# anibali/dsnt-pose2d

Measured on AMD Instinct MI355X. Metric: images/sec (train step, 256x256, 16 joints), higher is better.
Workload: dtype f32; 1 GPU; hg2 + DSNT + JS reg, 256x256 -> 64x64x16, batch 32 per GPU, RMSprop lr 2.5e-4, train step fwd+loss+bwd+optim; global_batch=32, parallelism=dp1, launches_fwd=212

## Files before the change

### dsnt-pose2d_amd/csrc/fwd1.h

```cpp
#pragma once
#include "conv_split.h"

struct Fwd1Plan {
    int ok;
    int cfg;
    int chunks;
    int nstages;
    int spw;
    int nwg;
    int lds;
};
Fwd1Plan dsnt_fwd1_plan(const dsnt_conv_geom* g, bool share);
```

### dsnt-pose2d_amd/csrc/fwd1.hip

```cpp
#include "fwd1.h"
#include <stdlib.h>

typedef unsigned f1_u32x4 __attribute__((ext_vector_type(4)));
typedef float f32x4 __attribute__((ext_vector_type(4)));

struct Fwd1P {
    const float* x; const float* in_scale; const float* in_shift; int in_relu;
    const unsigned short* wq; long wq_stride;
    const float* a_bound; const float* w_bound;
    const float* bias; const float* res; float* y; float* stats;
    OutBoundsP ob;
    int M, Cout, nstages, spw;
};

template <int KK, int CW, int NWV, bool PRO, bool RES>
__global__ __launch_bounds__(64 * NWV, 2) void fwd1_kernel(Fwd1P p) {
    constexpr int CC = 16 * CW * NWV;
    constexpr int NTHR = 64 * NWV;
    constexpr int KS = KK / 32;
    constexpr int PITCH = KK * 2 + 32;
    constexpr int PL = 32 * PITCH;
    constexpr int IMG = 2 * PL;
    constexpr int WLO = CC * PITCH;
    constexpr int K4 = KK / 4;
    constexpr int U = 32 * K4 / NTHR;
    constexpr int RSTEP = NTHR / K4;
    static_assert(U >= 1 && U * NTHR == 32 * K4, "staging units per thread");
    const unsigned OOB = 0xF0000000u;
    extern __shared__ __attribute__((aligned(16))) unsigned char f1_smem[];
    unsigned char* img = f1_smem;
    unsigned char* wlo = f1_smem + 2 * IMG;
// ... 94 lines not shown
        const int c = col0 + c0 + 16 * cw + lc;
        cb[cw] = p.bias ? p.bias[c] : 0.f;
        asc[cw] = p.ob.amax_bn ? p.ob.amax_scale[c] : 0.f;
        ash[cw] = p.ob.amax_bn ? p.ob.amax_shift[c] : 0.f;
    }
    const float am2lo = p.ob.amax_relu ? 0.f : -__builtin_inff();
    __syncthreads();
    transform(0);
    issue(s0 + 1);
    __syncthreads();

    float s1a[CW], s2a[CW];
#pragma unroll
    for (int cw = 0; cw < CW; ++cw) { s1a[cw] = 0.f; s2a[cw] = 0.f; }
    float am = 0.f, am2 = 0.f;
    const unsigned a_lane = (unsigned)(lc * PITCH + 16 * lg);
    const unsigned w_lane = (unsigned)(2 * IMG + (c0 + lc) * PITCH + 16 * lg);

    auto stage = [&](const int s) {
        const int buf = (s - s0) & 1;
        transform(buf ^ 1);
        issue(s + 2);
        __builtin_amdgcn_sched_barrier(0);
        const unsigned ib = (unsigned)(buf * IMG);
#pragma unroll
        for (int rt = 0; rt < 2; ++rt) {
            f32x4 acc[CW];
#pragma unroll
            for (int cw = 0; cw < CW; ++cw) acc[cw] = (f32x4){0.f, 0.f, 0.f, 0.f};
#pragma unroll
            for (int ks = 0; ks < KS; ++ks) {
                const unsigned ao = ib + (unsigned)(rt * 16 * PITCH + 64 * ks) + a_lane;
                const f16x8 d1 = *reinterpret_cast<const f16x8*>(f1_smem + ao);
                const f16x8 d2 = *reinterpret_cast<const f16x8*>(f1_smem + ao + PL);
#pragma unroll
                for (int cw = 0; cw < CW; ++cw) {
                    const f16x8 b2 = *reinterpret_cast<const f16x8*>(f1_smem + w_lane + cw * 16 * PITCH + 64 * ks);
                    acc[cw] = __builtin_amdgcn_mfma_f32_16x16x32_f16(d2, whi[ks][cw], acc[cw], 0, 0, 0);
                    acc[cw] = __builtin_amdgcn_mfma_f32_16x16x32_f16(d1, b2, acc[cw], 0, 0, 0);
                    acc[cw] = __builtin_amdgcn_mfma_f32_16x16x32_f16(d1, whi[ks][cw], acc[cw], 0, 0, 0);
                }
            }
            const unsigned obase = (unsigned)(s * 32 + 16 * rt) * (unsigned)ld * 4u + ylane;
#pragma unroll
            for (int cw = 0; cw < CW; ++cw) {
#pragma unroll
                for (int r = 0; r < 4; ++r) {
                    float v = acc[cw][r] * osc + cb[cw];
                    if (RES) v += rv[rt][cw][r];
                    __builtin_amdgcn_raw_buffer_store_b32(__float_as_uint(v), yr, obase + (unsigned)(cw * 64), (unsigned)(r * ld * 4), 0);
                    am = fmaxf(am, fabsf(v));
                    am2 = fmaxf(am2, fabsf(fmaxf(fmaf(v, asc[cw], ash[cw]), am2lo)));
                    s1a[cw] += v;
                    s2a[cw] = fmaf(v, v, s2a[cw]);
                }
            }
            issue_r(rt, s + 1);
        }
        __syncthreads();
    };
    stage(s0);
    for (int s = s0 + 1; s < s1; ++s) stage(s);

    if (p.stats) {
#pragma unroll
        for (int cw = 0; cw < CW; ++cw) {
            float a = s1a[cw], b = s2a[cw];
            a += __shfl_xor(a, 16, 64); b += __shfl_xor(b, 16, 64);
            a += __shfl_xor(a, 32, 64); b += __shfl_xor(b, 32, 64);
            if (lg == 0) {
                p.stats[((size_t)wg * 2 + 0) * ld + col0 + c0 + 16 * cw + lc] = a;
                p.stats[((size_t)wg * 2 + 1) * ld + col0 + c0 + 16 * cw + lc] = b;
            }
        }
    }
    if (p.ob.amax) amax_commit(am, p.ob.amax);
    if (p.ob.amax_bn) amax_commit(am2, p.ob.amax_bn, 1);
}

static int f1_enabled = -1;
struct F1Cfg { int cin, cout, cw, nwv, chunks; };
static const F1Cfg f1_cfgs[] = {
    {256, 128, 1, 8, 1},
    {128, 256, 2, 8, 1},
    {128, 128, 1, 8, 1},
    {64, 64, 1, 4, 1},
    {64, 128, 1, 8, 1},
    {256, 256, 1, 8, 2},
};

Fwd1Plan dsnt_fwd1_plan(const dsnt_conv_geom* g, bool share) {
    Fwd1Plan pl;
// ... 13 lines not shown
    const F1Cfg& c = f1_cfgs[cfg];
    const int cus = dsnt_device_cus();
    const int nstages = (int)(M / 32);
    int nwg = cus * (c.nwv == 4 ? 2 : 1) / c.chunks;
    if (share) nwg = nwg / 2 > 0 ? nwg / 2 : 1;
    if (c.chunks > 1) nwg = nwg / 8 * 8 > 0 ? nwg / 8 * 8 : nwg;
    if (nwg > nstages) nwg = nstages;
    const int spw = (nstages + nwg - 1) / nwg;
    nwg = (nstages + spw - 1) / spw;
    const int pitch = c.cin * 2 + 32;
    pl.ok = 1; pl.cfg = cfg; pl.nstages = nstages; pl.spw = spw; pl.nwg = nwg; pl.chunks = c.chunks;
    pl.lds = 2 * 2 * 32 * pitch + 16 * c.cw * c.nwv * pitch + 2 * c.cin * 4;
    return pl;
}

template <int KK, int CW, int NWV, bool PRO, bool RES>
static void f1_launch_k(const Fwd1Plan& pl, const Fwd1P& p, hipStream_t st) {
    DSNT_SET_MAX_LDS((fwd1_kernel<KK, CW, NWV, PRO, RES>), pl.lds);
    DSNT_LAUNCH((fwd1_kernel<KK, CW, NWV, PRO, RES>), dim3(pl.nwg, pl.chunks), dim3(64 * NWV), pl.lds, st, p);
}
template <int KK, int CW, int NWV>
static void f1_launch_cfg(const Fwd1Plan& pl, const Fwd1P& p, hipStream_t st) {
    const bool pro = p.in_scale != nullptr, res = p.res != nullptr;
    if (pro) { if (res) f1_launch_k<KK, CW, NWV, true, true>(pl, p, st); else f1_launch_k<KK, CW, NWV, true, false>(pl, p, st); }
    else { if (res) f1_launch_k<KK, CW, NWV, false, true>(pl, p, st); else f1_launch_k<KK, CW, NWV, false, false>(pl, p, st); }
}

extern "C" int dsnt_conv1x1_fwd_ok(const dsnt_conv_geom* g) { return dsnt_fwd1_plan(g, false).ok; }
extern "C" int dsnt_conv1x1_fwd_stats_rows(const dsnt_conv_geom* g, int in_relu_flags) {
    return dsnt_fwd1_plan(g, (in_relu_flags & DSNT_CONV_SHARE_CHIP) != 0).nwg;
// ... 16 lines not shown
    if (int e = out_bounds_fill(p.ob, tail, "dsnt_conv1x1_fwd_f16x3")) return e;
    p.x = x; p.in_scale = in_scale; p.in_shift = in_shift; p.in_relu = in_relu & 1;
    p.wq = (const unsigned short*)w_planes; p.wq_stride = plane_stride; p.a_bound = a_bound; p.w_bound = w_bound;
    p.bias = bias; p.res = res1; p.y = y; p.stats = stats_partial;
    p.M = g->N * g->H * g->W; p.Cout = g->Cout; p.nstages = pl.nstages; p.spw = pl.spw;
    hipStream_t st = (hipStream_t)stream;
    switch (pl.cfg) {
    case 0: case 5: f1_launch_cfg<256, 1, 8>(pl, p, st); break;
    case 1: f1_launch_cfg<128, 2, 8>(pl, p, st); break;
    case 2: f1_launch_cfg<128, 1, 8>(pl, p, st); break;
    case 3: f1_launch_cfg<64, 1, 4>(pl, p, st); break;
    default: f1_launch_cfg<64, 1, 8>(pl, p, st); break;
    }
    DSNT_CHECK_LAUNCH("dsnt_conv1x1_fwd_f16x3");
}
```

### dsnt-pose2d_amd/dsnt/_lib.py

```python
import ctypes as C
import os

import torch

_HERE = os.path.dirname(os.path.abspath(__file__))
LIB_PATH = os.environ.get('DSNT_HIP_LIB') or os.path.join(os.path.dirname(_HERE), 'csrc', 'libdsnt_hip.so')

P = C.c_void_p
I = C.c_int
L = C.c_int64
F = C.c_float
D = C.c_double


class ConvGeom(C.Structure):
    _fields_ = [(n, C.c_int) for n in
                ('N', 'H', 'W', 'Cin', 'Ho', 'Wo', 'Cout', 'R', 'S', 'stride', 'pad', 'dil')]


GP = C.POINTER(ConvGeom)


class BnBwdEpilogue(C.Structure):
    _fields_ = [('x', C.c_void_p), ('scale', C.c_void_p), ('shift', C.c_void_p), ('mean', C.c_void_p),
# ... 61 lines not shown
    'dsnt_conv_fwd_bf16x6_ex': [P, P, L, P, P, P, P, I, P, P, P, GP, BP, TP, P],
    'dsnt_conv_pack_dgrad': [P, P, I, I, I, I, P],
    'dsnt_conv_pack_dgrad_all': [P, I, P, P, P, L, P],
    'dsnt_conv_fwd_bf16x6': [P, P, L, P, P, P, P, I, P, P, P, GP, P],
    'dsnt_split_bf16x3': [P, P, L, P],
    'dsnt_conv_fwd_f16x3_ex': [P, P, L, P, P, P, P, P, P, I, P, P, P, GP, BP, TP, P],
    'dsnt_conv_fwd_f16x3_stream': [P, P, L, P, P, P, P, P, P, I, P, P, P, GP, BP, TP, P],
    'dsnt_amax': [P, L, P, P],
    'dsnt_split_f16x2': [P, P, L, L, P, P],
    'dsnt_f16_prep_weights': [P, I, I, P],
    'dsnt_f16_prep_bn_bounds': [P, I, P],
    'dsnt_conv_wgrad': [P, P, P, I, P, P, P, P, I, GP, P],
    'dsnt_conv_wgrad_bf16x6': [P, P, P, I, P, P, P, P, I, GP, P],
    'dsnt_conv_wgrad_f16x3': [P, P, P, I, P, P, P, P, I, P, P, GP, P],
    'dsnt_conv1x1_fwd_f16x3': [P, P, L, P, P, P, P, P, P, I, P, P, GP, TP, P],
    'dsnt_conv1x1_bwd_f16x3': [BP, P, AP, P, L, P, P, P, P, P, P, P, I, GP, P],
    'dsnt_conv_dgrad_f16x3_stream_apply': [P, AP, P, P, L, P, P, P, P, I, GP, BP, TP, P],
    'dsnt_wgrad_reduce_all': [P, I, I, P],
    'dsnt_conv_wgrad_group': [P, I, I, P],
    'dsnt_bn_stats': [P, P, L, I, P],
    'dsnt_bn_finalize': [P, I, L, I, P, P, P, P, F, F, I, P, P, P, P, P],
    'dsnt_bn_act_fwd': [P, P, P, I, P, L, I, P],
    'dsnt_bn_act_bwd_reduce': [P, P, P, P, P, P, I, P, L, I, P],
    'dsnt_bn_bwd_finalize': [P, I, L, I, P, P, I, P, P],
    'dsnt_bn_bwd_finalize_bound': [P, I, L, I, P, P, I, P, P, P, P, P],
    'dsnt_bn_eval_prep': [P, I, P],
    'dsnt_bn_act_bwd_apply': [P, P, P, P, P, P, P, I, P, I, L, I, P],
    'dsnt_bn_act_bwd_apply_amax': [P, P, P, P, P, P, P, I, P, I, L, I, P, P],
    'dsnt_bn_act_bwd_apply_pro': [P, P, P, P, P, P, P, I, P, P, I, P, I, P, I, L, I, P, P],
    'dsnt_stem4_fwd_f16x3': [P, P, L, P, P, P, P, P, GP, TP, P],
# ... 70 lines not shown
    'dsnt_conv_bf16x6_ok': (I, [GP]),
    'dsnt_conv_wgrad_bf16x6_ok': (I, [GP]),
    'dsnt_conv_wgrad_splits': (I, [GP]),
    'dsnt_conv_wgrad_halo_ok': (I, [GP]),
    'dsnt_conv_f16x3_route': (I, [GP, I]),
    'dsnt_conv_fwd_stream_ok': (I, [GP]),
    'dsnt_conv_fwd_stream_form': (I, [GP, I]),
    'dsnt_conv_dgrad_strided_ok': (I, [GP]),
    'dsnt_conv_dgrad_strided_tiles': (I, [GP]),
    'dsnt_conv_fwd_pro_ok': (I, [GP, I, I]),
    'dsnt_conv_wgrad_f16x3_splits': (I, [GP, I]),
    'dsnt_conv_wgrad_f16x3_ws_floats': (L, [GP, I]),
    'dsnt_conv_wgrad_ws_floats': (L, [GP]),
    'dsnt_conv1x1_fwd_ok': (I, [GP]),
    'dsnt_conv1x1_fwd_stats_rows': (I, [GP, I]),
    'dsnt_stem4_fwd_ok': (I, [GP]),
    'dsnt_stem4_fwd_stats_rows': (I, [GP]),
    'dsnt_conv1x1_bwd_ok': (I, [GP]),
    'dsnt_conv1x1_bwd_splits': (I, [GP, I]),
    'dsnt_conv1x1_bwd_ws_floats': (L, [GP, I]),
    'dsnt_conv_wgrad_desc_bytes': (I, []),
    'dsnt_conv_wgrad_desc': (I, [P, P, P, I, P, P, GP, P]),
    'dsnt_conv_wgrad_desc_f16x3': (I, [P, P, P, I, P, P, P, P, GP, P]),
    'dsnt_debug_set_timeline': (I, [P, I]),
}

_lib = None


def load():
# ... 50 lines not shown
```

### dsnt-pose2d_amd/dsnt/engine.py

```python
import ctypes as C
import os

import torch

from . import _lib
from ._lib import ConvGeom, BnBwdEpilogue, BnTail, BnPrologue, BnBwdApply

BN_EPS = 1e-5
BN_MOMENTUM = 0.1


class Act:
    __slots__ = ('buf', 'N', 'H', 'W', 'C', '_grad', 'stats', 'name', 'grad_amax', 'amax_tail', 'fold_ok',
                 'pending_apply', 'uses', 'gives_away', 'is_branch', 'grad_shared', 'pending_add', 'base', 'base_amax')

    def __init__(self, buf, name=''):
        self.buf = buf
        self.N, self.H, self.W, self.C = buf.shape
        self._grad = None
        self.base, self.base_amax = None, None
        self.stats = None
        self.amax_tail = None
        self.grad_amax = None
        self.fold_ok = False
        self.pending_apply = None
        self.uses = 0
        self.gives_away = False
        self.is_branch = False
        self.grad_shared = False
        self.pending_add = None
        self.name = name

    @property
    def M(self):
        return self.N * self.H * self.W

# ... 57 lines not shown
        self.side_stream = None
        self.wgrad_stream = None
        self.side_lanes = (1, 3)
        self.n_lanes = 3 + len(self.side_lanes) - 1
        self.chain_lanes = (0,) + self.side_lanes
        self.more_streams = ()
        self.wgrad_lane = 2 if (self.use_lanes and os.environ.get('DSNT_WGRAD_LANE', '1') != '0') else None
        self.wgrad_lane_rows = int(os.environ.get('DSNT_X_WGRAD_LANE_ROWS', '16000'))
        self.wgrad_lane_res = False
        self.wgrad_lane_from = self.chain_lanes
        self.conv3s = 'conv3s' not in os.environ.get('DSNT_OFF', '').replace('+', ',').split(',')
        self.bwd1 = 'bwd1' not in os.environ.get('DSNT_OFF', '').replace('+', ',').split(',')
        self.fwd1 = 'fwd1' not in os.environ.get('DSNT_OFF', '').replace('+', ',').split(',')
        self.fold3 = 'fold3' not in os.environ.get('DSNT_OFF', '').replace('+', ',').split(',')
        self.fold3_rows = int(os.environ.get('DSNT_X_FOLD3_ROWS', '16384'))
        self.stem4 = 'stem4' not in os.environ.get('DSNT_OFF', '').replace('+', ',').split(',')
        self.stage = os.environ.get('DSNT_STAGE', '0') == '1'
        self.stage_min_run = int(os.environ.get('DSNT_X_STAGE_MIN_RUN', '3'))
        self.stage_max_vgrid = int(os.environ.get('DSNT_X_STAGE_MAX_VGRID', '512'))
        self.stage_grid = int(os.environ.get('DSNT_X_STAGE_GRID', '64'))
        self.stage_census = []
        self._f16_w_stream = {}
        self.conv_share = True
        self.wgrad_share = True
        self._x = dict(kv.split('=') for kv in os.environ.get('DSNT_X', '').split(',') if '=' in kv)
        self.wgrad_narrow = self._x.get('wgrad_narrow', '1')
        self.share_grads = self._x.get('share_grads', '1') != '0'
        self.defer_res = self._x.get('defer_res', '1') != '0'
        self.flush_points = self._x.get('flush_points', '1') != '0'
        self.prep_split = self._x.get('prep_split', '1') != '0'
# ... 126 lines not shown
            return None
        got = self._famax_bn_of.get(id(t))
        if got is not None:
            return got[1] if got[0] is n else None
        slot = self._famax_slot()
        t.amax_bn, t.amax_scale, t.amax_shift = slot.data_ptr(), n.scale.data_ptr(), n.shift.data_ptr()
        t.amax_relu = 1 if n.relu else 0
        self._famax_bn_of[id(t)] = (n, slot)
        self._keep.append(t)
        return slot

    def f16_bn_bound_bwd(self, n):
        assert n.abound is not None, 'fp16x3 backward needs the BN bound its forward conv registered'
        return n.abound

    _PREP_CONSUMERS = ('dsnt_conv_fwd_f16x3_ex', 'dsnt_conv_fwd_f16x3_stream', 'dsnt_conv1x1_fwd_f16x3', 'dsnt_stem4_fwd_f16x3',
                       'dsnt_conv_fwd_bf16x6_ex', 'dsnt_conv_fwd_bf16x6')

    def emit_f16_prep(self, pos, head=()):
        side = 1 if (self.use_lanes and self.prep_on_side_lane and self.training) else 0
        saved, self.fwd = self.fwd, []
        saved_lane, self.lane = self.lane, side
        for fn, args, name, _ in head:
            self.fwd.append((fn, args, name, side))
        if self._f16_w_rows:
            t = torch.tensor(self._f16_w_rows, dtype=torch.int64).to(self.device)
            self._keep.append(t)
            self.f('dsnt_f16_prep_weights', t, len(self._f16_w_rows), 7)
        if self._f16_bn_rows:
            t = torch.tensor(self._f16_bn_rows, dtype=torch.int64).to(self.device)
            self._keep.append(t)
# ... 485 lines not shown
                self.b('dsnt_bn_act_bwd_apply_pro_base', da, x.buf, n.scale, n.shift, n.mean, n.invstd, part, tiles,
                       bn.ggamma, bn.gbeta, acc_p, coef, relu, base, buf, x.M, bn.C, x.grad_amax)
            else:
                self.b('dsnt_bn_act_bwd_apply_pro', da, x.buf, n.scale, n.shift, n.mean, n.invstd, part, tiles,
                       bn.ggamma, bn.gbeta, acc_p, coef, relu, buf, acc, x.M, bn.C, x.grad_amax)
        elif base is not None:
            self.b('dsnt_bn_act_bwd_apply_base', da, x.buf, n.scale, n.shift, n.mean, n.invstd, coef, relu,
                   base, buf, x.M, bn.C, x.grad_amax)
        elif x.grad_amax is not None:
            self.b('dsnt_bn_act_bwd_apply_amax', da, x.buf, n.scale, n.shift, n.mean, n.invstd, coef, relu,
                   buf, acc, x.M, bn.C, x.grad_amax)
        else:
            self.b('dsnt_bn_act_bwd_apply', da, x.buf, n.scale, n.shift, n.mean, n.invstd, coef, relu,
                   buf, acc, x.M, bn.C)

    def conv(self, src, p, res1=None, res2=None, want_stats=False, need_input_grad=True, name=''):
        normed = isinstance(src, Normed)
        x = src.x if normed else src
        g = self.geom(x, p)
        y = self.act(x.N, g.Ho, g.Wo, p.Cout, name)
        x.uses += 1
        for r in (res1, res2):
            if r is not None:
                r.uses += 1
                y.gives_away = True
        sc = src.scale if normed else None
        sh = src.shift if normed else None
        relu = 1 if (normed and src.relu) else 0
        if normed:
            self.check_lane(src)
        part, tail = None, None
        use6 = self._use6(g) and p.wq is not None
        x_amax_pre = None
        if use6 and p.wq16 is not None and p.R == 1 and res2 is None and self.fwd1:
            x_amax_pre = self.operand_amax_bn(src) if normed else self.operand_amax(x)
        f1 = bool(use6 and self.use_f16x3 and p.wq16 is not None and p.R == 1 and res2 is None and self.fwd1 and
                  ((self.training and normed) or x_amax_pre is not None) and self.lib.dsnt_conv1x1_fwd_ok(C.byref(g)))
        f1_shr = 2 if (f1 and self.lane != 0 and self.conv_share) else 0
        s4 = bool(use6 and self.use_f16x3 and self.stem4 and p.wq16 is not None and not normed and res1 is None and res2 is None and
                  self.lib.dsnt_stem4_fwd_ok(C.byref(g)))
        if want_stats and self.training:
            bm = 128 if use6 else self.lib.dsnt_conv_fwd_bm(C.byref(g))
            tiles = (self.lib.dsnt_conv1x1_fwd_stats_rows(C.byref(g), f1_shr) if f1 else
                     self.lib.dsnt_stem4_fwd_stats_rows(C.byref(g)) if s4 else (y.M + bm - 1) // bm)
            part = self.empty(tiles, 2, p.Cout)
            y.stats = (part, tiles)
        if use6 and self.use_f16x3:
            y.amax_tail = tail = BnTail()
        r1 = res1.buf if res1 is not None else None
        r2 = res2.buf if res2 is not None else None
        if self.use_f16x3 and self.training and normed:
            self.f16_bn_bound(src)
        x_amax = x_amax_pre
        if x_amax is None and use6 and p.wq16 is not None:
            x_amax = self.operand_amax_bn(src) if normed else self.operand_amax(x)
        use16 = use6 and self.use_f16x3 and p.wq16 is not None and ((self.training and normed) or x_amax is not None)
        if normed and (use16 or use6):
            self.materialize(src)
        if use16:
            st = self.stream_ok(p, g, y.M, res2)
            self.f16_weights(p, stream=st)
            ab = self.f16_bn_bound(src) if (normed and self.training) else x_amax
            shr = 2 if ((st or p.R == 1) and self.lane != 0 and self.conv_share) else 0
            if f1:
                e = self.f('dsnt_conv1x1_fwd_f16x3', x.buf, p.wq16, p.wq_stride, p.wb, ab, p.b, y.buf, sc, sh, relu | f1_shr, r1,
                           part, g, tail)
            elif s4:
                e = self.f('dsnt_stem4_fwd_f16x3', x.buf, p.wq16, p.wq_stride, p.wb, ab, p.b, y.buf, part, g, tail)
            else:
                e = self.f('dsnt_conv_fwd_f16x3_stream' if st else 'dsnt_conv_fwd_f16x3_ex', x.buf, p.wq16, p.wq_stride, p.wb, ab,
                           p.b, y.buf, sc, sh, relu | shr, r1, r2, part, g, None, tail)
            self.f16_uses.append((e, dict(kind='fwd', name=name, x=x.buf, sc=sc, sh=sh, relu=relu, a_bound=ab,
                                          w=p.w, w_bound=p.wb)))
        elif use6:
            self.f('dsnt_conv_fwd_bf16x6_ex', x.buf, p.wq, p.wq_stride, p.b, y.buf, sc, sh, relu, r1, r2, part, g,
                   None, tail)
        elif normed and src.pending is not None and self.lib.dsnt_conv_fwd_pro_ok(C.byref(g), src.pending[1], src.bn.C):
            spart, stiles = src.pending
            src.pending = None
# ... 300 lines not shown
            y.amax_tail = BnTail() if big else None
            self.f('dsnt_bn_act_fwd_stats', x.buf, n.scale, n.shift, 1 if n.relu else 0, y.buf, part, x.M, x.C, y.amax_tail)
            y.stats = (part, tiles)
        elif not self.training and big:
            y.amax_tail = BnTail()
            self.f('dsnt_bn_act_fwd_stats', x.buf, n.scale, n.shift, 1 if n.relu else 0, y.buf, None, x.M, x.C, y.amax_tail)
        else:
            self.f('dsnt_bn_act_fwd', x.buf, n.scale, n.shift, 1 if n.relu else 0, y.buf, x.M, x.C)
        if self.record:
            def backward():
                self._norm_backward(n, y.grad)
            self.on_backward(backward)
        return y

    def maxpool2(self, x, name=''):
        y = self.act(x.N, x.H // 2, x.W // 2, x.C, name)
        x.uses += 1
        idx = self.empty(x.N, x.H // 2, x.W // 2, x.C, dtype=torch.uint8)
        if self.training and self.fuse_op_stats:
            tiles = (y.M + 127) // 128
            part = self.empty(tiles, 2, x.C)
            y.amax_tail = BnTail() if (self.use_f16x3 and y.M >= self.bf16x6_min_rows) else None
            self.f('dsnt_maxpool2_fwd_stats', x.buf, y.buf, idx, part, x.N, x.H, x.W, x.C, y.amax_tail)
            y.stats = (part, tiles)
        elif not self.training and self.use_f16x3 and y.M >= self.bf16x6_min_rows:
            y.amax_tail = BnTail()
            self.f('dsnt_maxpool2_fwd_stats', x.buf, y.buf, idx, None, x.N, x.H, x.W, x.C, y.amax_tail)
        else:
            self.f('dsnt_maxpool2_fwd', x.buf, y.buf, idx, x.N, x.H, x.W, x.C)
        if self.record:
            def backward():
                add, x.pending_add = x.pending_add, None
                buf, acc = self.grad_target(x, amax=True, take_add=True)
                if add is not None:
# ... 128 lines not shown
```

### dsnt-pose2d_amd/dsnt/hourglass.py

```python
import os

import torch
import torch.nn as nn
from torch.autograd import Function

from . import _lib
from .engine import Tape, ConvParams, BnParams

EXPANSION = 2


def _ceil4(n):
    return (n + 3) // 4 * 4


class Arena:

    def __init__(self, module, device):
        self.device = device
        self.publish_scale = 1.0
        slots, off = [], 0
        skip = tuple(getattr(module, 'tape_exclude', ()))
        named = [(n, p) for n, p in module.named_parameters() if not (skip and n.startswith(skip))]
        bucket_of = getattr(module, 'param_bucket', lambda name: 0)
# ... 336 lines not shown
    expansion = EXPANSION

    def __init__(self, inplanes, planes, stride=1, downsample=None):
        super().__init__()
        self.bn1 = nn.BatchNorm2d(inplanes)
        self.conv1 = nn.Conv2d(inplanes, planes, kernel_size=1, bias=True)
        self.bn2 = nn.BatchNorm2d(planes)
        self.conv2 = nn.Conv2d(planes, planes, kernel_size=3, stride=stride, padding=1, bias=True)
        self.bn3 = nn.BatchNorm2d(planes)
        self.conv3 = nn.Conv2d(planes, planes * 2, kernel_size=1, bias=True)
        self.relu = nn.ReLU(inplace=True)
        self.downsample = downsample
        self.stride = stride
        self.out_channels = planes * 2

    def trace(self, t, x, P):
        skip = x
        if self.downsample is not None:
            skip = t.conv(x, P.conv(self.downsample[0]), name='ds')
        y = t.conv(t.norm(x, P.bn(self.bn1)), P.conv(self.conv1), want_stats=True, name='c1')
        y = t.conv(t.norm(y, P.bn(self.bn2)), P.conv(self.conv2), want_stats=True, name='c2')
        return t.conv(t.norm(y, P.bn(self.bn3)), P.conv(self.conv3), res1=skip, want_stats=True,
                      name='c3')


def _trace_seq(seq, t, x, P):
    for m in seq:
        x = m.trace(t, x, P)
    return x


class Hourglass(TapeModule):

    def __init__(self, block, num_blocks, planes, depth):
        super().__init__()
        self.depth = depth
        self.block = block
        self.upsample = nn.Upsample(scale_factor=2, mode='nearest')
        levels = []
        for i in range(depth):
            groups = [nn.Sequential(*[block(planes * block.expansion, planes) for _ in range(num_blocks)])
                      for _ in range(4 if i == 0 else 3)]
            levels.append(nn.ModuleList(groups))
# ... 4 lines not shown
        g = self.hg[n - 1]
        if t.record and t.use_lanes and t.fuse_join:
            side = t.side_lanes[n % len(t.side_lanes)]
            xb = t.branch(x, join=False)
            t.sync(0, side, bwd=False)
            pooled = t.maxpool2(x)

            def take_branch_gradient():
                t.sync_bwd(side, 0)
                if xb.grad is not None:
                    if x.grad is not None and x.pending_apply is None and t.share_grads:
                        t.add_later(x, xb.grad, xb.grad_amax)
                    else:
                        t.grad_identity(x, xb.grad, donate=True, g_amax=xb.grad_amax)
            t.on_backward(take_branch_gradient)
            low = _trace_seq(g[1], t, pooled, P)
            low = self._level(n - 1, t, low, P) if n > 1 else _trace_seq(g[3], t, low, P)
            low = _trace_seq(g[2], t, low, P)
            t.lane = side
            up1 = _trace_seq(g[0], t, xb, P)
            t.lane = 0
            t.sync(side, 0)
            return t.upsample2_add(up1, low)
        xb = t.branch(x)
        t.sync(0, 1)
        t.lane = 1 if t.use_lanes else 0
        up1 = _trace_seq(g[0], t, xb, P)
        t.lane = 0
        low = _trace_seq(g[1], t, t.maxpool2(x), P)
        low = self._level(n - 1, t, low, P) if n > 1 else _trace_seq(g[3], t, low, P)
        low = _trace_seq(g[2], t, low, P)
        t.sync(1, 0)
        return t.upsample2_add(up1, low)

    def trace(self, t, x, P):
        return self._level(self.depth, t, x, P)


class HourglassNet(TapeModule):
    supports_input_grad = True

    def __init__(self, block, num_stacks=2, num_blocks=4, num_classes=16):
        super().__init__()
        self.inplanes = 64
# ... 40 lines not shown
    def param_bucket(self, name):
        parts = name.split('.')
        if parts[0] in ('hg', 'res', 'fc', 'score', 'fc_', 'score_'):
            return 1 + int(parts[1])
        return 0

    def trace(self, t, x, P):
        if x.H % 64 != 0 or x.W % 64 != 0:
            raise RuntimeError('dsnt: hourglass input must be a multiple of 64 pixels '
                               '(stem /4, four 2x2 poolings), got %dx%d' % (x.H, x.W))
        t.mark_bucket(0)
        stem = P.conv(self.conv1)
        gi = getattr(t, 'want_input_grad', False)
        x = (None if gi else t.stem_s2d(x, stem)) or t.conv(x, stem, want_stats=True, need_input_grad=gi, name='stem')
        x = t.bn_act(x, P.bn(self.bn1), relu=True, name='stem_act')
        x = _trace_seq(self.layer1, t, x, P)
        x = t.maxpool2(x)
        x = _trace_seq(self.layer3, t, _trace_seq(self.layer2, t, x, P), P)
        outs = []
        for i in range(self.num_stacks):
            t.mark_bucket(1 + i)
            y = self.hg[i].trace(t, x, P)
            y = _trace_seq(self.res[i], t, y, P)
            y = t.conv(y, P.conv(self.fc[i][0]), want_stats=True, name='fc')
            yn = t.norm(y, P.bn(self.fc[i][1]), relu=True)
            score = t.conv(yn, P.conv(self.score[i]), name='score')
            if i < self.num_stacks - 1:
                f = t.conv(yn, P.conv(self.fc_[i]), name='fc_')
                x = t.conv(score, P.conv(self.score_[i]), res1=x, res2=f, want_stats=True, name='score_')
            outs.append(score)
        return outs
```

### include/dsnt_hip.h

```cpp
#ifndef DSNT_HIP_H
#define DSNT_HIP_H

#include <stdint.h>

#ifdef __cplusplus
extern "C" {
#endif

typedef enum {
    DSNT_OK = 0,
    DSNT_ERR_SHAPE = 1,
    DSNT_ERR_ALIGN = 2,
    DSNT_ERR_ARG = 3,
    DSNT_ERR_HIP = 4
} dsnt_status;

typedef struct {
    float* amax;
    float* amax_bn; const float* amax_scale; const float* amax_shift; int amax_relu, reserved;
} dsnt_out_bounds;

typedef struct dsnt_bn_prologue {
    const float* partial; int tiles, C;
    int64_t M;
// ... 153 lines not shown
                          const float* a_bound, const float* g_bound, const dsnt_conv_geom* g, void* stream);
int dsnt_conv_wgrad_desc_f16x3(const float* x, const float* in_scale, const float* in_shift, int in_relu,
                               const float* dy, float* ws, const float* a_bound, const float* g_bound,
                               const dsnt_conv_geom* g, void* desc_out);
int dsnt_conv_wgrad_halo_ok(const dsnt_conv_geom* g);
int dsnt_conv_f16x3_route(const dsnt_conv_geom* g, int wgrad);
int dsnt_conv_wgrad_f16x3_splits(const dsnt_conv_geom* g, int accumulate);
int64_t dsnt_conv_wgrad_f16x3_ws_floats(const dsnt_conv_geom* g, int accumulate);

int dsnt_conv1x1_fwd_ok(const dsnt_conv_geom* g);
int dsnt_conv1x1_fwd_stats_rows(const dsnt_conv_geom* g, int in_relu);
int dsnt_conv1x1_fwd_f16x3(const float* x, const void* w_planes, int64_t plane_stride, const float* w_bound,
                           const float* a_bound, const float* bias, float* y, const float* in_scale,
                           const float* in_shift, int in_relu, const float* res1, float* stats_partial,
                           const dsnt_conv_geom* g, const dsnt_out_bounds* tail, void* stream);
int dsnt_stem4_fwd_ok(const dsnt_conv_geom* g);
int dsnt_stem4_fwd_stats_rows(const dsnt_conv_geom* g);
int dsnt_stem4_fwd_f16x3(const float* x, const void* w_planes, int64_t plane_stride, const float* w_bound,
                         const float* a_bound, const float* bias, float* y, float* stats_partial,
                         const dsnt_conv_geom* g, const dsnt_out_bounds* tail, void* stream);


typedef struct {
    const float* y;
    const float* scale; const float* mean; const float* invstd;
    const float* coef;
} dsnt_bn_bwd_apply;
int dsnt_conv1x1_bwd_ok(const dsnt_conv_geom* g);
int dsnt_conv1x1_bwd_splits(const dsnt_conv_geom* g, int flags);
int64_t dsnt_conv1x1_bwd_ws_floats(const dsnt_conv_geom* g, int flags);
// ... 177 lines not shown
```

Baseline: 2914 images/sec.

## Fuse 2x2 maxpool into the 1x1 conv3 forward epilogue of bottlenecks

Adds a pooling variant of the 1x1 conv forward kernel. It holds the first row of each 2x2 window in registers and, once the second row is computed, writes the pooled max, the argmax index and the pooled statistics and bounds. Hourglass and stem bottlenecks that feed a maxpool now use it, and maxpool2 reuses the precomputed result instead of launching its own kernel. For layer1 the full-resolution output is dropped entirely ('drop' mode), which saves its write and the reread by the pool. The cost is more register pressure from the held rows, and stage counts per workgroup are rounded up to keep pool rows together, which may reduce parallelism.

```diff
diff --git a/dsnt-pose2d_amd/csrc/fwd1.h b/dsnt-pose2d_amd/csrc/fwd1.h
--- a/dsnt-pose2d_amd/csrc/fwd1.h
+++ b/dsnt-pose2d_amd/csrc/fwd1.h
@@ -11,3 +11,4 @@
     int lds;
 };
 Fwd1Plan dsnt_fwd1_plan(const dsnt_conv_geom* g, bool share);
+Fwd1Plan dsnt_fwd1_pool_plan(const dsnt_conv_geom* g, bool share, int* klog);
diff --git a/dsnt-pose2d_amd/csrc/fwd1.hip b/dsnt-pose2d_amd/csrc/fwd1.hip
--- a/dsnt-pose2d_amd/csrc/fwd1.hip
+++ b/dsnt-pose2d_amd/csrc/fwd1.hip
@@ -1,8 +1,17 @@
 #include "fwd1.h"
 #include <stdlib.h>
+#include <type_traits>
 
 typedef unsigned f1_u32x4 __attribute__((ext_vector_type(4)));
 typedef float f32x4 __attribute__((ext_vector_type(4)));
+
+template <int K, int N, class F>
+__device__ __forceinline__ void f1_dispatch(const int i, F&& f) {
+    if constexpr (K < N) {
+        if (i == K) f(std::integral_constant<int, K>{});
+        else f1_dispatch<K + 1, N>(i, f);
+    }
+}
 
 struct Fwd1P {
     const float* x; const float* in_scale; const float* in_shift; int in_relu;
@@ -11,10 +20,14 @@
     const float* bias; const float* res; float* y; float* stats;
     OutBoundsP ob;
     int M, Cout, nstages, spw;
+    float* yp; unsigned char* pidx; float* pstats;
+    OutBoundsP pob;
+    int klog;
 };
 
-template <int KK, int CW, int NWV, bool PRO, bool RES>
+template <int KK, int CW, int NWV, bool PRO, bool RES, int POOL = 0>
 __global__ __launch_bounds__(64 * NWV, 2) void fwd1_kernel(Fwd1P p) {
+    constexpr int KMAX = POOL ? (CW == 1 ? 4 : 2) : 0;
     constexpr int CC = 16 * CW * NWV;
     constexpr int NTHR = 64 * NWV;
     constexpr int KS = KK / 32;
@@ -139,6 +152,60 @@
 #pragma unroll
     for (int cw = 0; cw < CW; ++cw) { s1a[cw] = 0.f; s2a[cw] = 0.f; }
     float am = 0.f, am2 = 0.f;
+    float hv[POOL ? 2 * KMAX : 1][CW][4];
+    float ps1[CW], ps2[CW], pasc[CW], pash[CW];
+    float pam = 0.f, pam2 = 0.f;
+#pragma unroll
+    for (int cw = 0; cw < CW; ++cw) {
+        const int c = col0 + c0 + 16 * cw + lc;
+        ps1[cw] = 0.f; ps2[cw] = 0.f;
+        pasc[cw] = (POOL && p.pob.amax_bn) ? p.pob.amax_scale[c] : 0.f;
+        pash[cw] = (POOL && p.pob.amax_bn) ? p.pob.amax_shift[c] : 0.f;
+#pragma unroll
+        for (int k = 0; k < (POOL ? 2 * KMAX : 1); ++k)
+#pragma unroll
+            for (int r = 0; r < 4; ++r) hv[k][cw][r] = 0.f;
+    }
+    const float pam2lo = (POOL && p.pob.amax_relu) ? 0.f : -__builtin_inff();
+    const __amdgpu_buffer_rsrc_t ypr = __builtin_amdgcn_make_buffer_rsrc(POOL ? p.yp : p.y, 0, (int)((size_t)(p.M / 4) * ld * 4u), 0x00020000);
+    const __amdgpu_buffer_rsrc_t pir = __builtin_amdgcn_make_buffer_rsrc(POOL ? (void*)p.pidx : (void*)p.y, 0, (int)((size_t)(p.M / 4) * ld), 0x00020000);
+    const bool w16 = p.klog < 0;
+    const int klog = w16 ? 0 : p.klog;
+    auto pool_half = [&](const int s, const int rt, const float (&vv)[CW][4]) {
+        const int row = s >> klog, seg = s & ((1 << klog) - 1);
+        const bool fin = w16 ? rt == 1 : (row & 1) != 0;
+        const int hs = w16 ? 0 : 2 * seg + rt;
+        const unsigned pp = w16 ? (unsigned)s * 8u : ((unsigned)(((row >> 1) << klog) + seg) * 16u + 8u * rt);
+        const unsigned pbase = (pp + 2u * lg) * (unsigned)ld + (unsigned)(col0 + c0 + lc);
+        f1_dispatch<0, (POOL ? 2 * KMAX : 1)>(hs, [&](auto slot) {
+            constexpr int k = decltype(slot)::value;
+            if (!fin) {
+#pragma unroll
+                for (int cw = 0; cw < CW; ++cw)
+#pragma unroll
+                    for (int r = 0; r < 4; ++r) hv[k][cw][r] = vv[cw][r];
+                return;
+            }
+#pragma unroll
+            for (int cw = 0; cw < CW; ++cw)
+#pragma unroll
+                for (int h = 0; h < 2; ++h) {
+                    float m = hv[k][cw][2 * h];
+                    unsigned q = 0;
+                    const float v1 = hv[k][cw][2 * h + 1], v2 = vv[cw][2 * h], v3 = vv[cw][2 * h + 1];
+                    if (v1 > m || v1 != v1) { m = v1; q = 1; }
+                    if (v2 > m || v2 != v2) { m = v2; q = 2; }
+                    if (v3 > m || v3 != v3) { m = v3; q = 3; }
+                    const unsigned o = pbase + (unsigned)(h * ld + 16 * cw);
+                    __builtin_amdgcn_raw_buffer_store_b32(__float_as_uint(m), ypr, o * 4u, 0, 0);
+                    __builtin_amdgcn_raw_buffer_store_b8((unsigned char)q, pir, o, 0, 0);
+                    pam = fmaxf(pam, fabsf(m));
+                    pam2 = fmaxf(pam2, fabsf(fmaxf(fmaf(m, pasc[cw], pash[cw]), pam2lo)));
+                    ps1[cw] += m;
+                    ps2[cw] = fmaf(m, m, ps2[cw]);
+                }
+        });
+    };
     const unsigned a_lane = (unsigned)(lc * PITCH + 16 * lg);
     const unsigned w_lane = (unsigned)(2 * IMG + (c0 + lc) * PITCH + 16 * lg);
 
@@ -167,12 +234,15 @@
                 }
             }
             const unsigned obase = (unsigned)(s * 32 + 16 * rt) * (unsigned)ld * 4u + ylane;
+            float vv[POOL ? CW : 1][4];
 #pragma unroll
             for (int cw = 0; cw < CW; ++cw) {
 #pragma unroll
                 for (int r = 0; r < 4; ++r) {
                     float v = acc[cw][r] * osc + cb[cw];
                     if (RES) v += rv[rt][cw][r];
+                    if (POOL) vv[cw][r] = v;
+                    if (POOL == 2) continue;
                     __builtin_amdgcn_raw_buffer_store_b32(__float_as_uint(v), yr, obase + (unsigned)(cw * 64), (unsigned)(r * ld * 4), 0);
                     am = fmaxf(am, fabsf(v));
                     am2 = fmaxf(am2, fabsf(fmaxf(fmaf(v, asc[cw], ash[cw]), am2lo)));
@@ -180,6 +250,7 @@
                     s2a[cw] = fmaf(v, v, s2a[cw]);
                 }
             }
+            if constexpr (POOL != 0) pool_half(s, rt, vv);
             issue_r(rt, s + 1);
         }
         __syncthreads();
@@ -201,6 +272,23 @@
     }
     if (p.ob.amax) amax_commit(am, p.ob.amax);
     if (p.ob.amax_bn) amax_commit(am2, p.ob.amax_bn, 1);
+    if (POOL) {
+        if (p.pstats) {
+#pragma unroll
+            for (int cw = 0; cw < CW; ++cw) {
+                float a = ps1[cw], b = ps2[cw];
+                a += __shfl_xor(a, 16, 64); b += __shfl_xor(b, 16, 64);
+                a += __shfl_xor(a, 32, 64); b += __shfl_xor(b, 32, 64);
+                if (lg == 0) {
+                    p.pstats[((size_t)wg * 2 + 0) * ld + col0 + c0 + 16 * cw + lc] = a;
+                    p.pstats[((size_t)wg * 2 + 1) * ld + col0 + c0 + 16 * cw + lc] = b;
+                }
+            }
+        }
+        __syncthreads();
+        if (p.pob.amax) amax_commit(pam, p.pob.amax);
+        if (p.pob.amax_bn) amax_commit(pam2, p.pob.amax_bn, 1);
+    }
 }
 
 static int f1_enabled = -1;
@@ -244,6 +332,32 @@
     return pl;
 }
 
+Fwd1Plan dsnt_fwd1_pool_plan(const dsnt_conv_geom* g, bool share, int* klog) {
+    Fwd1Plan pl = dsnt_fwd1_plan(g, share);
+    static int pool_enabled = -1;
+    if (pool_enabled < 0) pool_enabled = dsnt_kernel_off("pool1") ? 0 : 1;
+    if (!pl.ok || !pool_enabled) { pl.ok = 0; return pl; }
+    const int kmax = pl.cfg == 4 ? 4 : pl.cfg == 1 ? 2 : 0;
+    const int W = g->W;
+    const bool wok = W == 16 || ((W == 32 || W == 64 || W == 128) && W / 32 <= kmax);
+    if (!kmax || !wok || g->H % 2 != 0 || pl.chunks != 1) { pl.ok = 0; return pl; }
+    int kl = -1;
+    if (W >= 32) {
+        kl = W == 32 ? 0 : W == 64 ? 1 : 2;
+        const int unit = 2 << kl;
+        pl.spw = (pl.spw + unit - 1) / unit * unit;
+        pl.nwg = (pl.nstages + pl.spw - 1) / pl.spw;
+    }
+    if (klog) *klog = kl;
+    return pl;
+}
+
+template <int KK, int CW, int NWV, int POOL>
+static void f1_launch_pool(const Fwd1Plan& pl, const Fwd1P& p, hipStream_t st) {
+    DSNT_SET_MAX_LDS((fwd1_kernel<KK, CW, NWV, true, true, POOL>), pl.lds);
+    DSNT_LAUNCH((fwd1_kernel<KK, CW, NWV, true, true, POOL>), dim3(pl.nwg, pl.chunks), dim3(64 * NWV), pl.lds, st, p);
+}
+
 template <int KK, int CW, int NWV, bool PRO, bool RES>
 static void f1_launch_k(const Fwd1Plan& pl, const Fwd1P& p, hipStream_t st) {
     DSNT_SET_MAX_LDS((fwd1_kernel<KK, CW, NWV, PRO, RES>), pl.lds);
@@ -290,3 +404,39 @@
     }
     DSNT_CHECK_LAUNCH("dsnt_conv1x1_fwd_f16x3");
 }
+
+extern "C" int dsnt_conv1x1_fwd_pool_ok(const dsnt_conv_geom* g) { return dsnt_fwd1_pool_plan(g, false, nullptr).ok; }
+extern "C" int dsnt_conv1x1_fwd_pool_stats_rows(const dsnt_conv_geom* g, int in_relu_flags) {
+    return dsnt_fwd1_pool_plan(g, (in_relu_flags & DSNT_CONV_SHARE_CHIP) != 0, nullptr).nwg;
+}
+
+extern "C" int dsnt_conv1x1_fwd_pool_f16x3(const float* x, const void* w_planes, int64_t plane_stride, const float* w_bound,
+                                           const float* a_bound, const float* bias, float* y, const float* in_scale,
+                                           const float* in_shift, int in_relu, const float* res1, float* stats_partial,
+                                           float* y_pool, uint8_t* idx, float* pool_stats, const dsnt_conv_geom* g,
+                                           const dsnt_out_bounds* tail, const dsnt_out_bounds* pool_tail, void* stream) {
+    DSNT_REQUIRE(x && w_planes && w_bound && a_bound && y_pool && idx && g, DSNT_ERR_ARG, "dsnt_conv1x1_fwd_pool_f16x3: bad argument");
+    DSNT_REQUIRE(in_scale && in_shift && res1, DSNT_ERR_ARG,
+                 "dsnt_conv1x1_fwd_pool_f16x3: needs the BatchNorm operand vectors and a residual (conv3 of a Bottleneck)");
+    DSNT_REQUIRE(y || (!stats_partial && !tail), DSNT_ERR_ARG,
+                 "dsnt_conv1x1_fwd_pool_f16x3: without y there are no full-resolution statistics or bounds");
+    int klog = -1;
+    const Fwd1Plan pl = dsnt_fwd1_pool_plan(g, (in_relu & DSNT_CONV_SHARE_CHIP) != 0, &klog);
+    DSNT_REQUIRE(pl.ok, DSNT_ERR_SHAPE, "dsnt_conv1x1_fwd_pool_f16x3: geometry not supported (dsnt_conv1x1_fwd_pool_ok)");
+    DSNT_REQUIRE(dsnt_aligned16(x) && dsnt_aligned16(w_planes) && (!y || dsnt_aligned16(y)) && dsnt_aligned16(res1) &&
+                 dsnt_aligned16(y_pool) && dsnt_aligned16(in_scale) && dsnt_aligned16(in_shift) && plane_stride % 8 == 0,
+                 DSNT_ERR_ALIGN, "dsnt_conv1x1_fwd_pool_f16x3: 16-byte alignment required");
+    Fwd1P p;
+    memset(&p, 0, sizeof(p));
+    if (int e = out_bounds_fill(p.ob, tail, "dsnt_conv1x1_fwd_pool_f16x3")) return e;
+    if (int e = out_bounds_fill(p.pob, pool_tail, "dsnt_conv1x1_fwd_pool_f16x3")) return e;
+    p.x = x; p.in_scale = in_scale; p.in_shift = in_shift; p.in_relu = in_relu & 1;
+    p.wq = (const unsigned short*)w_planes; p.wq_stride = plane_stride; p.a_bound = a_bound; p.w_bound = w_bound;
+    p.bias = bias; p.res = res1; p.y = y; p.stats = stats_partial;
+    p.M = g->N * g->H * g->W; p.Cout = g->Cout; p.nstages = pl.nstages; p.spw = pl.spw;
+    p.yp = y_pool; p.pidx = idx; p.pstats = pool_stats; p.klog = klog;
+    hipStream_t st = (hipStream_t)stream;
+    if (pl.cfg == 1) { if (y) f1_launch_pool<128, 2, 8, 1>(pl, p, st); else f1_launch_pool<128, 2, 8, 2>(pl, p, st); }
+    else { if (y) f1_launch_pool<64, 1, 8, 1>(pl, p, st); else f1_launch_pool<64, 1, 8, 2>(pl, p, st); }
+    DSNT_CHECK_LAUNCH("dsnt_conv1x1_fwd_pool_f16x3");
+}
diff --git a/dsnt-pose2d_amd/dsnt/_lib.py b/dsnt-pose2d_amd/dsnt/_lib.py
--- a/dsnt-pose2d_amd/dsnt/_lib.py
+++ b/dsnt-pose2d_amd/dsnt/_lib.py
@@ -99,6 +99,7 @@
     'dsnt_conv_wgrad_bf16x6': [P, P, P, I, P, P, P, P, I, GP, P],
     'dsnt_conv_wgrad_f16x3': [P, P, P, I, P, P, P, P, I, P, P, GP, P],
     'dsnt_conv1x1_fwd_f16x3': [P, P, L, P, P, P, P, P, P, I, P, P, GP, TP, P],
+    'dsnt_conv1x1_fwd_pool_f16x3': [P, P, L, P, P, P, P, P, P, I, P, P, P, P, P, GP, TP, TP, P],
     'dsnt_conv1x1_bwd_f16x3': [BP, P, AP, P, L, P, P, P, P, P, P, P, I, GP, P],
     'dsnt_conv_dgrad_f16x3_stream_apply': [P, AP, P, P, L, P, P, P, P, I, GP, BP, TP, P],
     'dsnt_wgrad_reduce_all': [P, I, I, P],
@@ -199,6 +200,8 @@
     'dsnt_conv_wgrad_ws_floats': (L, [GP]),
     'dsnt_conv1x1_fwd_ok': (I, [GP]),
     'dsnt_conv1x1_fwd_stats_rows': (I, [GP, I]),
+    'dsnt_conv1x1_fwd_pool_ok': (I, [GP]),
+    'dsnt_conv1x1_fwd_pool_stats_rows': (I, [GP, I]),
     'dsnt_stem4_fwd_ok': (I, [GP]),
     'dsnt_stem4_fwd_stats_rows': (I, [GP]),
     'dsnt_conv1x1_bwd_ok': (I, [GP]),
diff --git a/dsnt-pose2d_amd/dsnt/engine.py b/dsnt-pose2d_amd/dsnt/engine.py
--- a/dsnt-pose2d_amd/dsnt/engine.py
+++ b/dsnt-pose2d_amd/dsnt/engine.py
@@ -11,7 +11,7 @@
 
 
 class Act:
-    __slots__ = ('buf', 'N', 'H', 'W', 'C', '_grad', 'stats', 'name', 'grad_amax', 'amax_tail', 'fold_ok',
+    __slots__ = ('buf', 'N', 'H', 'W', 'C', '_grad', 'stats', 'name', 'grad_amax', 'amax_tail', 'fold_ok', 'pooled',
                  'pending_apply', 'uses', 'gives_away', 'is_branch', 'grad_shared', 'pending_add', 'base', 'base_amax')
 
     def __init__(self, buf, name=''):
@@ -20,6 +20,7 @@
         self._grad = None
         self.base, self.base_amax = None, None
         self.stats = None
+        self.pooled = None
         self.amax_tail = None
         self.grad_amax = None
         self.fold_ok = False
@@ -107,6 +108,7 @@
         self.fwd1 = 'fwd1' not in os.environ.get('DSNT_OFF', '').replace('+', ',').split(',')
         self.fold3 = 'fold3' not in os.environ.get('DSNT_OFF', '').replace('+', ',').split(',')
         self.fold3_rows = int(os.environ.get('DSNT_X_FOLD3_ROWS', '16384'))
+        self.pool1 = self.fwd1 and 'pool1' not in os.environ.get('DSNT_OFF', '').replace('+', ',').split(',')
         self.stem4 = 'stem4' not in os.environ.get('DSNT_OFF', '').replace('+', ',').split(',')
         self.stage = os.environ.get('DSNT_STAGE', '0') == '1'
         self.stage_min_run = int(os.environ.get('DSNT_X_STAGE_MIN_RUN', '3'))
@@ -263,7 +265,8 @@
         assert n.abound is not None, 'fp16x3 backward needs the BN bound its forward conv registered'
         return n.abound
 
-    _PREP_CONSUMERS = ('dsnt_conv_fwd_f16x3_ex', 'dsnt_conv_fwd_f16x3_stream', 'dsnt_conv1x1_fwd_f16x3', 'dsnt_stem4_fwd_f16x3',
+    _PREP_CONSUMERS = ('dsnt_conv_fwd_f16x3_ex', 'dsnt_conv_fwd_f16x3_stream', 'dsnt_conv1x1_fwd_f16x3', 'dsnt_conv1x1_fwd_pool_f16x3',
+                       'dsnt_stem4_fwd_f16x3',
                        'dsnt_conv_fwd_bf16x6_ex', 'dsnt_conv_fwd_bf16x6')
 
     def emit_f16_prep(self, pos, head=()):
@@ -779,16 +782,14 @@
             self.b('dsnt_bn_act_bwd_apply', da, x.buf, n.scale, n.shift, n.mean, n.invstd, coef, relu,
                    buf, acc, x.M, bn.C)
 
-    def conv(self, src, p, res1=None, res2=None, want_stats=False, need_input_grad=True, name=''):
+    def conv(self, src, p, res1=None, res2=None, want_stats=False, need_input_grad=True, name='', pool=None):
         normed = isinstance(src, Normed)
         x = src.x if normed else src
         g = self.geom(x, p)
-        y = self.act(x.N, g.Ho, g.Wo, p.Cout, name)
         x.uses += 1
         for r in (res1, res2):
             if r is not None:
                 r.uses += 1
-                y.gives_away = True
         sc = src.scale if normed else None
         sh = src.shift if normed else None
         relu = 1 if (normed and src.relu) else 0
@@ -802,15 +803,26 @@
         f1 = bool(use6 and self.use_f16x3 and p.wq16 is not None and p.R == 1 and res2 is None and self.fwd1 and
                   ((self.training and normed) or x_amax_pre is not None) and self.lib.dsnt_conv1x1_fwd_ok(C.byref(g)))
         f1_shr = 2 if (f1 and self.lane != 0 and self.conv_share) else 0
+        f1p = bool(f1 and pool in ('keep', 'drop') and self.pool1 and normed and res1 is not None and
+                   self.lib.dsnt_conv1x1_fwd_pool_ok(C.byref(g)))
+        drop = f1p and pool == 'drop'
+        if drop:
+            y = Act(torch.empty(1, device=self.device).expand(x.N, g.Ho, g.Wo, p.Cout), name)
+            self.acts.append(y)
+        else:
+            y = self.act(x.N, g.Ho, g.Wo, p.Cout, name)
+        y.gives_away = res1 is not None or res2 is not None
         s4 = bool(use6 and self.use_f16x3 and self.stem4 and p.wq16 is not None and not normed and res1 is None and res2 is None and
                   self.lib.dsnt_stem4_fwd_ok(C.byref(g)))
         if want_stats and self.training:
             bm = 128 if use6 else self.lib.dsnt_conv_fwd_bm(C.byref(g))
-            tiles = (self.lib.dsnt_conv1x1_fwd_stats_rows(C.byref(g), f1_shr) if f1 else
+            tiles = (self.lib.dsnt_conv1x1_fwd_pool_stats_rows(C.byref(g), f1_shr) if f1p else
+                     self.lib.dsnt_conv1x1_fwd_stats_rows(C.byref(g), f1_shr) if f1 else
                      self.lib.dsnt_stem4_fwd_stats_rows(C.byref(g)) if s4 else (y.M + bm - 1) // bm)
-            part = self.empty(tiles, 2, p.Cout)
-            y.stats = (part, tiles)
-        if use6 and self.use_f16x3:
+            if not drop:
+                part = self.empty(tiles, 2, p.Cout)
+                y.stats = (part, tiles)
+        if use6 and self.use_f16x3 and not drop:
             y.amax_tail = tail = BnTail()
         r1 = res1.buf if res1 is not None else None
         r2 = res2.buf if res2 is not None else None
@@ -827,7 +839,19 @@
             self.f16_weights(p, stream=st)
             ab = self.f16_bn_bound(src) if (normed and self.training) else x_amax
             shr = 2 if ((st or p.R == 1) and self.lane != 0 and self.conv_share) else 0
-            if f1:
+            if f1p:
+                yp = self.act(x.N, g.Ho // 2, g.Wo // 2, p.Cout, name + '_pool')
+                idx = self.empty(x.N, g.Ho // 2, g.Wo // 2, p.Cout, dtype=torch.uint8)
+                ppart = None
+                if self.training and self.fuse_op_stats:
+                    ptiles = self.lib.dsnt_conv1x1_fwd_pool_stats_rows(C.byref(g), f1_shr)
+                    ppart = self.empty(ptiles, 2, p.Cout)
+                    yp.stats = (ppart, ptiles)
+                yp.amax_tail = BnTail() if yp.M >= self.bf16x6_min_rows else None
+                y.pooled = (yp, idx)
+                e = self.f('dsnt_conv1x1_fwd_pool_f16x3', x.buf, p.wq16, p.wq_stride, p.wb, ab, p.b, None if drop else y.buf, sc, sh,
+                           relu | f1_shr, r1, part, yp.buf, idx, ppart, g, tail, yp.amax_tail)
+            elif f1:
                 e = self.f('dsnt_conv1x1_fwd_f16x3', x.buf, p.wq16, p.wq_stride, p.wb, ab, p.b, y.buf, sc, sh, relu | f1_shr, r1,
                            part, g, tail)
             elif s4:
@@ -1158,10 +1182,15 @@
         return y
 
     def maxpool2(self, x, name=''):
-        y = self.act(x.N, x.H // 2, x.W // 2, x.C, name)
         x.uses += 1
-        idx = self.empty(x.N, x.H // 2, x.W // 2, x.C, dtype=torch.uint8)
-        if self.training and self.fuse_op_stats:
+        if x.pooled is not None:
+            y, idx = x.pooled
+        else:
+            y = self.act(x.N, x.H // 2, x.W // 2, x.C, name)
+            idx = self.empty(x.N, x.H // 2, x.W // 2, x.C, dtype=torch.uint8)
+        if x.pooled is not None:
+            pass
+        elif self.training and self.fuse_op_stats:
             tiles = (y.M + 127) // 128
             part = self.empty(tiles, 2, x.C)
             y.amax_tail = BnTail() if (self.use_f16x3 and y.M >= self.bf16x6_min_rows) else None
diff --git a/dsnt-pose2d_amd/dsnt/hourglass.py b/dsnt-pose2d_amd/dsnt/hourglass.py
--- a/dsnt-pose2d_amd/dsnt/hourglass.py
+++ b/dsnt-pose2d_amd/dsnt/hourglass.py
@@ -374,19 +374,19 @@
         self.stride = stride
         self.out_channels = planes * 2
 
-    def trace(self, t, x, P):
+    def trace(self, t, x, P, pool=None):
         skip = x
         if self.downsample is not None:
             skip = t.conv(x, P.conv(self.downsample[0]), name='ds')
         y = t.conv(t.norm(x, P.bn(self.bn1)), P.conv(self.conv1), want_stats=True, name='c1')
         y = t.conv(t.norm(y, P.bn(self.bn2)), P.conv(self.conv2), want_stats=True, name='c2')
         return t.conv(t.norm(y, P.bn(self.bn3)), P.conv(self.conv3), res1=skip, want_stats=True,
-                      name='c3')
-
-
-def _trace_seq(seq, t, x, P):
-    for m in seq:
-        x = m.trace(t, x, P)
+                      name='c3', pool=pool)
+
+
+def _trace_seq(seq, t, x, P, pool=None):
+    for i, m in enumerate(seq):
+        x = m.trace(t, x, P, pool=pool) if (pool and i == len(seq) - 1 and isinstance(m, Bottleneck)) else m.trace(t, x, P)
     return x
 
 
@@ -421,7 +421,7 @@
                     else:
                         t.grad_identity(x, xb.grad, donate=True, g_amax=xb.grad_amax)
             t.on_backward(take_branch_gradient)
-            low = _trace_seq(g[1], t, pooled, P)
+            low = _trace_seq(g[1], t, pooled, P, pool='keep' if n > 1 else None)
             low = self._level(n - 1, t, low, P) if n > 1 else _trace_seq(g[3], t, low, P)
             low = _trace_seq(g[2], t, low, P)
             t.lane = side
@@ -434,7 +434,7 @@
         t.lane = 1 if t.use_lanes else 0
         up1 = _trace_seq(g[0], t, xb, P)
         t.lane = 0
-        low = _trace_seq(g[1], t, t.maxpool2(x), P)
+        low = _trace_seq(g[1], t, t.maxpool2(x), P, pool='keep' if n > 1 else None)
         low = self._level(n - 1, t, low, P) if n > 1 else _trace_seq(g[3], t, low, P)
         low = _trace_seq(g[2], t, low, P)
         t.sync(1, 0)
@@ -505,9 +505,9 @@
         gi = getattr(t, 'want_input_grad', False)
         x = (None if gi else t.stem_s2d(x, stem)) or t.conv(x, stem, want_stats=True, need_input_grad=gi, name='stem')
         x = t.bn_act(x, P.bn(self.bn1), relu=True, name='stem_act')
-        x = _trace_seq(self.layer1, t, x, P)
+        x = _trace_seq(self.layer1, t, x, P, pool='drop')
         x = t.maxpool2(x)
-        x = _trace_seq(self.layer3, t, _trace_seq(self.layer2, t, x, P), P)
+        x = _trace_seq(self.layer3, t, _trace_seq(self.layer2, t, x, P), P, pool='keep')
         outs = []
         for i in range(self.num_stacks):
             t.mark_bucket(1 + i)
diff --git a/include/dsnt_hip.h b/include/dsnt_hip.h
--- a/include/dsnt_hip.h
+++ b/include/dsnt_hip.h
@@ -191,6 +191,13 @@
                            const float* a_bound, const float* bias, float* y, const float* in_scale,
                            const float* in_shift, int in_relu, const float* res1, float* stats_partial,
                            const dsnt_conv_geom* g, const dsnt_out_bounds* tail, void* stream);
+int dsnt_conv1x1_fwd_pool_ok(const dsnt_conv_geom* g);
+int dsnt_conv1x1_fwd_pool_stats_rows(const dsnt_conv_geom* g, int in_relu);
+int dsnt_conv1x1_fwd_pool_f16x3(const float* x, const void* w_planes, int64_t plane_stride, const float* w_bound,
+                                const float* a_bound, const float* bias, float* y, const float* in_scale,
+                                const float* in_shift, int in_relu, const float* res1, float* stats_partial,
+                                float* y_pool, uint8_t* idx, float* pool_stats, const dsnt_conv_geom* g,
+                                const dsnt_out_bounds* tail, const dsnt_out_bounds* pool_tail, void* stream);
 int dsnt_stem4_fwd_ok(const dsnt_conv_geom* g);
 int dsnt_stem4_fwd_stats_rows(const dsnt_conv_geom* g);
 int dsnt_stem4_fwd_f16x3(const float* x, const void* w_planes, int64_t plane_stride, const float* w_bound,
```

New measurement: 2944 images/sec (median of 6 runs). 1.01x the previous value.
